# ml-unito/PartitionedLS.jl

Measured on NVIDIA B200. Metric: opt_fit_orthant_nnls_solves_per_sec, higher is better.
Workload: dtype f64

## Files before the change

partitionedls.jl_b200/csrc/nnls5.cu:

```cuda
#include "common.cuh"

namespace pls {
namespace {

constexpr int H5_BYTES_ = 192;
constexpr int SG_FREE5 = 2;
constexpr unsigned char ST_INO = 1;
constexpr unsigned char ST_PAS = 2;
constexpr unsigned char ST_BLK = 4;
constexpr unsigned char ST_FAST = 8;
#define SYNC5() __syncthreads()

__device__ __forceinline__ void dmma5(double &d0, double &d1, double a, double b) {
  asm("mma.sync.aligned.m8n8k4.row.col.f64.f64.f64.f64 {%0,%1}, {%2}, {%3}, {%0,%1};\n"
      : "+d"(d0), "+d"(d1) : "d"(a), "d"(b));
}
__device__ __forceinline__ double rcp5(double x) {
  double r;
  asm("rcp.approx.ftz.f64 %0, %1;" : "=d"(r) : "d"(x));
  double e = fma(-x, r, 1.0);
  r = fma(r, e, r);
  e = fma(-x, r, 1.0);
  return fma(r, e, r);
}
__device__ __forceinline__ double wsum5(double v) {
#pragma unroll
  for (int o = 16; o; o >>= 1) v += __shfl_xor_sync(0xffffffffu, v, o);
  return v;
}
__device__ __forceinline__ double wmax5(double v) {
#pragma unroll
  for (int o = 16; o; o >>= 1) v = fmax(v, __shfl_xor_sync(0xffffffffu, v, o));
  return v;
}
__host__ __device__ constexpr int t2_doubles(int nr) { return ((nr / 8) * (nr / 8 + 1) / 2) * 64; }
__device__ __forceinline__ int t2_idx(int i, int j) {
  const int ti = i >> 3, tj = j >> 3;
  return ((((ti * (ti + 1)) >> 1) + tj) << 6) + ((i & 7) << 3) + (j & 7);
}
__device__ __forceinline__ double t2_get(const double *T2, int i, int j) { return i >= j ? T2[t2_idx(i, j)] : T2[t2_idx(j, i)]; }
__device__ __forceinline__ void t2_set(double *T2, int i, int j, double v) {
  const int a = i > j ? i : j, b = i > j ? j : i;
  const int x = t2_idx(a, b);
  T2[x] = v;
  if ((a >> 3) == (b >> 3)) T2[x - ((a & 7) << 3) - (b & 7) + ((b & 7) << 3) + (a & 7)] = v;
}
__device__ __forceinline__ int pan5(int row, int col) { return (row << 3) + (col ^ ((row & 2) << 1)); }

struct Sh5 {
  double *T2;
  double *v;
  double *Pp, *Wp;
  double *yv;
  double *D;
  double *gd;
  double *red;
  int4 *binfo;
  int *ctl;
  short *slot;
  short *rvar;
  short *lst;
  short *lstE;
  short *lstB;
  unsigned short *tmap;
  signed char *sg;
  unsigned char *st;
  unsigned char *grp;
  unsigned char *mk;
};
enum { C_NS = 0, C_OK, C_CNT, C_N, C_NJ, C_NP, C_NLV, C_FLAG };

__host__ __device__ inline size_t sh5_bytes(int NR, int ld1) {
  const int ntl = (NR / 8) * (NR / 8 + 1) / 2;
  return H5_BYTES_ + sizeof(double) * ((size_t)t2_doubles(NR) + ld1 + 16 * (size_t)NR + NR + 64 + 8 + 32 + 16) + sizeof(int) * 16 +
         sizeof(short) * (2 * (size_t)ld1 + 2 * (size_t)NR + 8 + ((ntl + 3) & ~3)) + 3 * (size_t)ld1 + NR + 16 + 16;
}

__device__ __forceinline__ Sh5 make_sh5(int NR, int ld1) {
  extern __shared__ __align__(16) unsigned char smem_raw5[];
  const int ntl = (NR / 8) * (NR / 8 + 1) / 2;
  Sh5 s;
  double *dp = reinterpret_cast<double *>(smem_raw5 + H5_BYTES_);
  s.T2 = dp; dp += t2_doubles(NR);
  s.Pp = dp; dp += 8 * NR;
  s.Wp = dp; dp += 8 * NR;
  s.yv = dp; dp += NR;
  s.D = dp; dp += 64;
  s.gd = dp; dp += 8;
  s.red = dp; dp += 32;
  s.binfo = reinterpret_cast<int4 *>(dp); dp += 16;
  int *ip = reinterpret_cast<int *>(dp);
  s.ctl = ip; ip += 16;
  short *sp = reinterpret_cast<short *>(ip);
  s.rvar = sp; sp += NR;
  s.lstE = sp; sp += NR;
  s.lstB = sp; sp += 8;
  s.tmap = reinterpret_cast<unsigned short *>(sp); sp += (ntl + 3) & ~3;
  s.mk = reinterpret_cast<unsigned char *>(sp);
  dp = reinterpret_cast<double *>(smem_raw5 + ((static_cast<int>(s.mk - smem_raw5) + NR + 15) & ~15));
  s.v = dp; dp += ld1;
  sp = reinterpret_cast<short *>(dp);
  s.slot = sp; sp += ld1;
  s.lst = sp; sp += ld1;
  signed char *cp = reinterpret_cast<signed char *>(sp);
  s.sg = cp; cp += ld1;
  s.st = reinterpret_cast<unsigned char *>(cp); cp += ld1;
  s.grp = reinterpret_cast<unsigned char *>(cp);
  return s;
}

struct H5 {
  double *T1;
  const double *T1r;
  double *Pg;
  const double *G;
  const unsigned long long *gmask;
  int ld1, nr, Mp, ldg;
  int cold_fused;
  int gen;
  int pad0, pad1;
  unsigned long long cnt[10];
  double yy, cmax;
  double max_viol;
};
enum { H_SWEEP = 0, H_STREAM, H_SUMS, H_SUMP2, H_ITER, H_BLK, H_REBUILD, H_FOLD, H_DRIFT, H_NOCONV };
constexpr int H5_BYTES = H5_BYTES_;
static_assert(sizeof(H5) <= H5_BYTES, "header size");
__device__ __forceinline__ H5 &hdr5() {
  extern __shared__ __align__(16) unsigned char smem_raw5[];
  return *reinterpret_cast<H5 *>(smem_raw5);
}

template <int T>
__device__ __forceinline__ double bmax5(const Sh5 &s, double v) {
  constexpr int NW = T / 32;
  v = wmax5(v);
  if ((threadIdx.x & 31) == 0) s.red[threadIdx.x >> 5] = v;
  SYNC5();
  double r = s.red[0];
#pragma unroll
  for (int i = 1; i < NW; ++i) r = fmax(r, s.red[i]);
  SYNC5();
  return r;
}

template <int T>
__device__ __forceinline__ void set_block5(const Sh5 &s, int nb, int slot) {
  const int tid = threadIdx.x;
  const H5 &h = hdr5();
  const int g = h.gen;
  if (g == 1) {
    #pragma unroll 1
    for (int k = tid; k < h.nr; k += T) s.mk[k] = 0;
    SYNC5();
  }
  if (tid < nb) {
    const int tc = slot >> 3, c7 = slot & 7;
    s.lstB[tid] = (short)slot;
    s.binfo[tid] = make_int4(slot, (tc << 6) + c7, (((tc * (tc + 1)) >> 1) << 6) + (c7 << 3), 0);
    s.mk[slot] = (unsigned char)g;
  }
}

template <int T, int NR>
__device__ __noinline__ int t2_block(int n, int nb, int nlv, bool test, bool flip) {
  H5 &h = hdr5();
  const int gen = h.gen;
  const Sh5 s = make_sh5(NR, h.ld1);
  constexpr int NW = T / 32;
  const int tid = threadIdx.x, lane = tid & 31, wid = tid >> 5;
  const int fr = lane >> 2, fk = lane & 3;
  const int ntr = (n + 7) >> 3;
  const short *B = s.lstB;
  if (tid >= 32 || T == 32) {
    constexpr int TG = T == 32 ? 32 : T - 32;
#pragma unroll 1
    for (int row = T == 32 ? tid : tid - 32; row < ntr * 8; row += TG) {
      const int tr = row >> 3, r7 = row & 7;
      const int rbase = (((tr * (tr + 1)) >> 1) << 6) + (r7 << 3), rowt = (tr << 6) + r7;
      const int sw = (row & 2) << 1, pb = row << 3;
#pragma unroll 1
      for (int q = 0; q < 8; ++q) {
        double val = 0.0;
        if (row < n && q < nb) { const int4 bi = s.binfo[q]; val = s.T2[row >= bi.x ? rbase + bi.y : bi.z + rowt]; }
        s.Pp[pb + (q ^ sw)] = val;
      }
    }
  }
  if (tid < 32) {
    if (lane < 8) {
      s.gd[lane] = (test && lane >= nlv && lane < nb) ? 1e-13 * __ldg(h.G + (size_t)h.ldg * s.rvar[B[lane]] + s.rvar[B[lane]]) : 0.0;
    }
    const int i = lane >> 2, j0 = (lane & 3) << 1;
    double e0 = (i < nb && j0 < nb) ? t2_get(s.T2, B[i], B[j0]) : (i == j0 ? 1.0 : 0.0);
    double e1 = (i < nb && j0 + 1 < nb) ? t2_get(s.T2, B[i], B[j0 + 1]) : (i == j0 + 1 ? 1.0 : 0.0);
    int bad = nb;
#pragma unroll 1
    for (int k = 0; k < nb; ++k) {
      __syncwarp();
      s.D[i * 8 + j0] = e0; s.D[i * 8 + j0 + 1] = e1;
      __syncwarp();
      const double pk0 = s.D[k * 8 + j0], pk1 = s.D[k * 8 + j0 + 1], cik = s.D[i * 8 + k], pkk = s.D[k * 8 + k];
      const bool good = k < nlv ? pkk < 0.0 : (test ? pkk > s.gd[k] : pkk > 0.0);
      if (!good && bad == nb) bad = k;
      const double d = rcp5(pkk), fct = cik * d;
      const bool rowk = i == k;
      double n0 = rowk ? pk0 * d : fma(-fct, pk0, e0);
      double n1 = rowk ? pk1 * d : fma(-fct, pk1, e1);
      if (j0 == k) n0 = rowk ? d : -fct;
      if (j0 + 1 == k) n1 = rowk ? d : -fct;
      e0 = n0; e1 = n1;
    }
    __syncwarp();
    s.D[i * 8 + j0] = e0; s.D[i * 8 + j0 + 1] = e1;
    if (lane == 0) s.ctl[C_OK] = bad == nb ? nb : (bad < nlv ? -1 : bad);
  }
  SYNC5();
  const int res = s.ctl[C_OK];
  if (tid == 0) h.gen = gen == 255 ? 1 : gen + 1;
  if (res != nb) { SYNC5(); return res; }
  #pragma unroll 1
  for (int ti = wid; ti < ntr; ti += NW) {
    double c0 = 0.0, c1 = 0.0;
    dmma5(c0, c1, s.Pp[pan5(ti * 8 + fr, fk)], s.D[fk * 8 + fr]);
    dmma5(c0, c1, s.Pp[pan5(ti * 8 + fr, 4 + fk)], s.D[(4 + fk) * 8 + fr]);
    *reinterpret_cast<double2 *>(s.Wp + pan5(ti * 8 + fr, 2 * fk)) = make_double2(c0, c1);
  }
  SYNC5();
  {
    const int ntl = (ntr * (ntr + 1)) >> 1;
    int q = (ntl * wid) / NW;
    const int q1 = (ntl * (wid + 1)) / NW;
    const int t0 = s.tmap[q];
    int ti = t0 >> 8, tj = t0 & 255;
    const int la0 = pan5(fr, fk), la1 = pan5(fr, 4 + fk);
    double2 *cp = reinterpret_cast<double2 *>(s.T2 + (q << 6) + fr * 8 + 2 * fk);
    const double *pw = s.Wp + (ti << 6), *pp = s.Pp + (tj << 6);
    double a0 = -pw[la0], a1 = -pw[la1];
#pragma unroll 1
    for (; q < q1; ++q) {
      double2 c0 = *cp;
      dmma5(c0.x, c0.y, a0, pp[la0]);
      dmma5(c0.x, c0.y, a1, pp[la1]);
      *cp = c0;
      cp += 32; pp += 64;
      if (++tj > ti) { ++ti; tj = 0; pp = s.Pp; pw += 64; a0 = -pw[la0]; a1 = -pw[la1]; }
    }
  }
  SYNC5();
#pragma unroll 1
  for (int row = tid; row < n; row += T) {
    if (s.mk[row] == (unsigned char)gen) continue;
    const int tr = row >> 3, r7 = row & 7;
    const int rbase = (((tr * (tr + 1)) >> 1) << 6) + (r7 << 3), rowt = (tr << 6) + r7;
    const int sw = (row & 2) << 1, pb = row << 3;
#pragma unroll 1
    for (int q = 0; q < nb; ++q) {
      const int4 bi = s.binfo[q];
      const int tc = bi.x >> 3;
      const double w0 = s.Wp[pb + (q ^ sw)];
      const double val = q < nlv ? -w0 : w0;
      if (tr >= tc) s.T2[rbase + bi.y] = val;
      if (tr <= tc) s.T2[bi.z + rowt] = val;
    }
  }
#pragma unroll 1
  for (int e = tid; e < 64; e += T) {
    const int i = e >> 3, j = e & 7;
    if (i < nb && j <= i) { const double val = s.D[i * 8 + j]; t2_set(s.T2, B[i], B[j], ((i < nlv) == (j < nlv)) ? -val : val); }
  }
  if (flip && tid < nb) s.st[s.rvar[B[tid]]] ^= ST_PAS;
  SYNC5();
  if (tid == 0) { h.cnt[H_SWEEP] += nb; h.cnt[H_SUMP2] += ((unsigned long long)(n * n) * nb) >> 2; }
  return nb;
}

template <int T, int NR>
__device__ __noinline__ bool t2_rebuild(int n) {
  const H5 &h = hdr5();
  const Sh5 s = make_sh5(NR, h.ld1);
  constexpr int NW = T / 32;
  const int tid = threadIdx.x, lane = tid & 31, wid = tid >> 5;
  #pragma unroll 1
  for (int i = wid; i < n; i += NW) {
    const double *row = h.T1r + (size_t)h.ld1 * s.rvar[i];
    #pragma unroll 1
    for (int j = lane; j <= i; j += 32) t2_set(s.T2, i, j, __ldcg(row + s.rvar[j]));
  }
  if (tid < 32) {
    int cnt = 0, nlv = 0;
    #pragma unroll 1
    for (int pass = 0; pass < 2; ++pass) {
      #pragma unroll 1
      for (int k0 = 1; k0 < n; k0 += 32) {
        const int k = k0 + lane;
        bool take = false;
        if (k < n) { const unsigned char f = s.st[s.rvar[k]]; const bool pas = f & ST_PAS, ino = f & ST_INO; take = pas != ino && (pass == 0 ? !pas : pas); }
        const unsigned bal = __ballot_sync(0xffffffffu, take);
        if (take) s.lst[cnt + __popc(bal & ((1u << lane) - 1))] = (short)k;
        cnt += __popc(bal);
      }
      if (pass == 0) nlv = cnt;
    }
    if (lane == 0) { s.ctl[C_CNT] = cnt; s.ctl[C_NLV] = nlv; }
  }
  SYNC5();
  const int cnt = s.ctl[C_CNT], nlv = s.ctl[C_NLV];
  #pragma unroll 1
  for (int q0 = 0; q0 < cnt; q0 += 8) {
    const int nb = min(8, cnt - q0);
    set_block5<T>(s, nb, tid < nb ? s.lst[q0 + tid] : 0);
    SYNC5();
    if (t2_block<T, NR>(n, nb, max(0, min(nb, nlv - q0)), false, false) != nb) return false;
  }
  return true;
}

template <int NR>
__device__ __noinline__ int window_reset() {
  const H5 &h = hdr5();
  const Sh5 s = make_sh5(NR, h.ld1);
  const int tid = threadIdx.x;
  const int Mp = h.Mp;
  if (tid < 32) {
    const int lane = tid;
    if (lane == 0) s.rvar[0] = (short)Mp;
    int base = 1;
    #pragma unroll 1
    for (int m0 = 0; m0 < Mp; m0 += 32) {
      const int m = m0 + lane;
      bool keep = false;
      if (m < Mp) {
        const unsigned char f = s.st[m];
        keep = (f & ST_FAST) || (((f & ST_PAS) != 0) != ((f & ST_INO) != 0));
      }
      const unsigned bal = __ballot_sync(0xffffffffu, keep);
      if (m < Mp) {
        if (keep) { const int k = base + __popc(bal & ((1u << lane) - 1)); s.rvar[k] = (short)m; s.slot[m] = (short)k; }
        else s.slot[m] = -1;
      }
      base += __popc(bal);
    }
    if (lane == 0) s.ctl[C_N] = base;
  }
  SYNC5();
  return s.ctl[C_N];
}

template <int T, int NR>
__device__ __noinline__ int t2_compact(int n) {
  const H5 &h = hdr5();
  const Sh5 s = make_sh5(NR, h.ld1);
  const int tid = threadIdx.x;
  double *scr = h.Pg + 8 * (size_t)h.ld1;
  short *old = s.lst;
  if (tid < 32) {
    const int lane = tid;
    if (lane == 0) old[0] = 0;
    int base = 1;
    #pragma unroll 1
    for (int k0 = 1; k0 < n; k0 += 32) {
      const int k = k0 + lane;
      bool keep = false; int m = 0;
      if (k < n) {
        m = s.rvar[k];
        const unsigned char f = s.st[m];
        keep = (f & ST_FAST) || (((f & ST_PAS) != 0) != ((f & ST_INO) != 0));
      }
      const unsigned bal = __ballot_sync(0xffffffffu, keep);
      const int kn = base + __popc(bal & ((1u << lane) - 1));
      __syncwarp();
      if (k < n) {
        if (keep) { old[kn] = (short)k; s.rvar[kn] = (short)m; s.slot[m] = (short)kn; }
        else s.slot[m] = -1;
      }
      __syncwarp();
      base += __popc(bal);
    }
    if (lane == 0) s.ctl[C_N] = base;
  }
  SYNC5();
  const int nn = s.ctl[C_N];
  if (nn == n) return n;
  #pragma unroll 1
  for (int idx = tid; idx < nn * nn; idx += T) {
    const int a = idx / nn, b = idx - a * nn;
    if (b <= a) __stcg(scr + idx, t2_get(s.T2, old[a], old[b]));
  }
  __threadfence_block();
  SYNC5();
  #pragma unroll 1
  for (int idx = tid; idx < nn * nn; idx += T) {
    const int a = idx / nn, b = idx - a * nn;
    if (b <= a) t2_set(s.T2, a, b, __ldcg(scr + idx));
  }
  SYNC5();
// ... 212 lines not shown
          __stcg(reinterpret_cast<double2 *>(h.T1 + (size_t)(ri[u] * 8 + fr) * ld1 + rj[u] * 8 + 2 * fk), c[u]);
          if (ri[u] != rj[u]) {
            double *mp = h.T1 + (size_t)(rj[u] * 8 + 2 * fk) * ld1 + ri[u] * 8 + fr;
            __stcg(mp, c[u].x); __stcg(mp + ld1, c[u].y);
          }
        }
      }
    }
  }
  SYNC5();
  #pragma unroll 1
  for (int idx = tid; idx < ld1 * 8; idx += T) {
    const int i = idx >> 3, q = idx & 7;
    if (q < nb) {
      const double val = (s.st[B[q]] & ST_PAS) ? FW[pan5(i, q)] : -FW[pan5(i, q)];
      __stcg(h.T1 + (size_t)ld1 * B[q] + i, val);
      __stcg(h.T1 + (size_t)ld1 * i + B[q], val);
    }
  }
  SYNC5();
  #pragma unroll 1
  for (int e = tid; e < 64; e += T) {
    const int i = e >> 3, j = e & 7;
    if (i < nb && j < nb) {
      const double ei = (s.st[B[i]] & ST_PAS) ? 1.0 : -1.0, ej = (s.st[B[j]] & ST_PAS) ? 1.0 : -1.0;
      __stcg(h.T1 + (size_t)ld1 * B[i] + B[j], -ei * ej * s.D[i * 8 + j]);
    }
  }
  SYNC5();
  if (tid < nb) { const int m = B[tid]; const unsigned char f = s.st[m]; s.st[m] = (f & ST_PAS) ? (unsigned char)(f | ST_INO) : (unsigned char)(f & ~ST_INO); }
  if (tid == 0) { h.T1r = h.T1; h.cnt[H_SUMP2] += 2ull * ld1 * ld1; h.cnt[H_FOLD]++; }
  SYNC5();
  return true;
}

template <int T, int NR>
__device__ __noinline__ void fold_fused5(int n) {
  H5 &h = hdr5();
  const Sh5 s = make_sh5(NR, h.ld1);
  constexpr int NW = T / 32;
  const int tid = threadIdx.x, lane = tid & 31, wid = tid >> 5;
  const int fr = lane >> 2, fk = lane & 3;
  const int ld1 = h.ld1, nt = ld1 >> 3;
  const int ntr = (n + 7) >> 3, nk = ntr << 3;
  double *PR = h.Pg + 8 * (size_t)ld1, *ZT = PR + (size_t)ld1 * h.nr;
  int *roff = reinterpret_cast<int *>(s.Wp);
  const bool own = h.T1r == h.T1;
  const double *rows = own ? PR : h.T1r;
  #pragma unroll 1
  for (int k = tid; k < nk; k += T) {
    double e = 0.0;
    if (k >= 1 && k < n) { const unsigned char f = s.st[s.rvar[k]]; const bool pas = f & ST_PAS, ino = f & ST_INO; if (pas != ino) e = pas ? 1.0 : -1.0; }
    s.yv[k] = e;
    roff[k] = e != 0.0 ? (own ? k : (int)s.rvar[k]) * ld1 : 0;
  }
  SYNC5();
  if (own) {
    #pragma unroll 1
    for (int k = 0; k < n; ++k) {
      if (k > 0 && s.yv[k] == 0.0) continue;
      const double *src = h.T1 + (size_t)ld1 * (s.yv[k] != 0.0 ? s.rvar[k] : 0);
      #pragma unroll 1
      for (int j = tid; j < ld1; j += T) PR[(size_t)k * ld1 + j] = __ldcg(src + j);
    }
    __threadfence_block();
    SYNC5();
  }
  constexpr int NTQ = 12;
#pragma unroll 1
  for (int tj = wid; tj < nt; tj += NW) {
    const double *pa = rows + tj * 8 + fr;
    double2 acc[NTQ];
#pragma unroll
    for (int u = 0; u < NTQ; ++u) acc[u] = make_double2(0.0, 0.0);
    double a0 = s.yv[fk] * __ldcg(pa + roff[fk]), a1 = s.yv[4 + fk] * __ldcg(pa + roff[4 + fk]);
#pragma unroll 1
    for (int tk = 0; tk < ntr; ++tk) {
      double n0 = 0.0, n1 = 0.0;
      if (tk + 1 < ntr) { const int k = (tk + 1) * 8 + fk; n0 = s.yv[k] * __ldcg(pa + roff[k]); n1 = s.yv[k + 4] * __ldcg(pa + roff[k + 4]); }
#pragma unroll
      for (int tq = 0; tq < NTQ; ++tq) {
        if (tq < ntr) {
          double b0, b1;
          if (tk >= tq) { const double *tp = s.T2 + ((((tk * (tk + 1)) >> 1) + tq) << 6); b0 = tp[fk * 8 + fr]; b1 = tp[(4 + fk) * 8 + fr]; }
          else { const double *tp = s.T2 + ((((tq * (tq + 1)) >> 1) + tk) << 6); b0 = tp[fr * 8 + fk]; b1 = tp[fr * 8 + 4 + fk]; }
          dmma5(acc[tq].x, acc[tq].y, a0, b0); dmma5(acc[tq].x, acc[tq].y, a1, b1);
        }
      }
      a0 = n0; a1 = n1;
    }
#pragma unroll
    for (int tq = 0; tq < NTQ; ++tq)
      if (tq < ntr) {
        const int k = tq * 8 + 2 * fk;
        *reinterpret_cast<double2 *>(ZT + (size_t)(tj * 8 + fr) * nk + k) = make_double2(acc[tq].x * s.yv[k], acc[tq].y * s.yv[k + 1]);
      }
  }
  __threadfence_block();
  SYNC5();
  constexpr int CH = 5;
  {
    const int ntl = (nt * (nt + 1)) >> 1;
    int q = (ntl * wid) / NW;
    const int q1 = (ntl * (wid + 1)) / NW;
    int ti = 0;
    while (((ti + 1) * (ti + 2)) >> 1 <= q) ++ti;
    int tj = q - ((ti * (ti + 1)) >> 1);
    #pragma unroll 1
    for (; q < q1; ++q) {
      double2 c = __ldcg(reinterpret_cast<const double2 *>(h.T1r + (size_t)(ti * 8 + fr) * ld1 + tj * 8 + 2 * fk));
      const double *za = ZT + (size_t)(ti * 8 + fr) * nk + fk, *pb = rows + tj * 8 + fr;
#pragma unroll 1
      for (int t0 = 0; t0 < ntr; t0 += CH) {
        double z0[CH], z1[CH], p0[CH], p1[CH];
#pragma unroll
        for (int u = 0; u < CH; ++u) {
          const bool live = t0 + u < ntr;
          const int k = (t0 + u) * 8 + fk;
          z0[u] = live ? za[(t0 + u) * 8] : 0.0; z1[u] = live ? za[(t0 + u) * 8 + 4] : 0.0;
          p0[u] = live ? __ldcg(pb + roff[k]) : 0.0; p1[u] = live ? __ldcg(pb + roff[k + 4]) : 0.0;
        }
#pragma unroll
        for (int u = 0; u < CH; ++u) { dmma5(c.x, c.y, z0[u], p0[u]); dmma5(c.x, c.y, z1[u], p1[u]); }
      }
      __stcg(reinterpret_cast<double2 *>(h.T1 + (size_t)(ti * 8 + fr) * ld1 + tj * 8 + 2 * fk), c);
      if (ti != tj) {
        double *mp = h.T1 + (size_t)(tj * 8 + 2 * fk) * ld1 + ti * 8 + fr;
        __stcg(mp, c.x); __stcg(mp + ld1, c.y);
      }
      if (++tj > ti) { ++ti; tj = 0; }
    }
  }
  SYNC5();
  #pragma unroll 1
  for (int k = 1; k < n; ++k) {
    const double e = s.yv[k];
    if (e == 0.0) continue;
    const int var = s.rvar[k];
    #pragma unroll 1
    for (int j = tid; j < ld1; j += T) {
      const double val = -e * ZT[(size_t)j * nk + k];
      __stcg(h.T1 + (size_t)ld1 * var + j, val);
      __stcg(h.T1 + (size_t)ld1 * j + var, val);
    }
  }
  SYNC5();
  #pragma unroll 1
  for (int idx = tid; idx < n * n; idx += T) {
    const int a = idx / n, b = idx - a * n;
    __stcg(h.T1 + (size_t)ld1 * s.rvar[a] + s.rvar[b], t2_get(s.T2, a, b));
  }
  SYNC5();
  #pragma unroll 1
  for (int k = tid; k < n; k += T) {
    if (k >= 1 && s.yv[k] != 0.0) { const int m = s.rvar[k]; const unsigned char f = s.st[m]; s.st[m] = (f & ST_PAS) ? (unsigned char)(f | ST_INO) : (unsigned char)(f & ~ST_INO); }
  }
  if (tid == 0) { h.T1r = h.T1; h.cnt[H_SUMP2] += 2ull * ld1 * ld1 * (unsigned long long)ntr / 8 + (unsigned long long)ld1 * nk * nk / 2; h.cnt[H_FOLD]++; }
  SYNC5();
}

template <int T, int NR>
__device__ __noinline__ int fold5(int n, bool cold_mode) {
  const H5 &h = hdr5();
  const Sh5 s = make_sh5(NR, h.ld1);
  const int tid = threadIdx.x;
  if (cold_mode) n = t2_compact<T, NR>(n);
  short *B = s.lstE;
  if (tid < 32) {
// ... 64 lines not shown
      a0 = fma(-h.G[(size_t)h.ldg * s.lst[t] + m], wf[t], a0);
      a1 = fma(-h.G[(size_t)h.ldg * s.lst[t + 1] + m], wf[t + 1], a1);
    }
    if (t < np) a0 = fma(-h.G[(size_t)h.ldg * s.lst[t] + m], wf[t], a0);
    const double rv = a0 + a1;
    const int sg = s.sg[m];
    const unsigned char f = s.st[m];
    if (f & ST_PAS) mx = fmax(mx, fabs(rv));
    else if (sg == SG_FREE5) mx = fmax(mx, fabs(rv));
    else if (sg != 0 && !(f & ST_BLK)) mx = fmax(mx, (double)sg * rv);
  }
  return bmax5<T>(s, mx);
}

template <int T, int NR, int NQ>
__device__ __forceinline__ bool solve5(const Sh5 s, int &n_win, bool cold_mode, bool &t2_fresh) {
  const int tid = threadIdx.x;
  H5 &h = hdr5();
  const int Mp = h.Mp;
  const double cmax = h.cmax;
  const double told = 1e-12 * cmax;
  int t_best = Mp + 1, pbar = 3, iters = 0, rebuilt = 0;
  #pragma unroll 1
  for (;;) {
    #pragma unroll 1
    for (;;) {
      const int n = n_win;
      int nl = 0, ne = 0, mx = -1;
      {
        constexpr int NW = T / 32;
        const int lane = tid & 31, wid = tid >> 5;
        int4 *ri = reinterpret_cast<int4 *>(s.red);
        #pragma unroll 1
        for (int k0 = 1; k0 < n; k0 += T) {
          const int k = k0 + tid;
          int f = 0, m = -1;
          if (k < n) {
            m = s.rvar[k];
            const double val = s.T2[t2_idx(k, 0)];
            const int sg = s.sg[m];
            const unsigned char fl = s.st[m];
            if (fl & ST_PAS) { if (sg != SG_FREE5 && (sg == 0 || (double)sg * val < 0.0)) f = 1; }
            else if (!(fl & ST_BLK) && sg != 0 && (sg == SG_FREE5 ? fabs(val) > told : (double)sg * val > told)) f = 2;
          }
          const unsigned bl = __ballot_sync(0xffffffffu, f == 1), be = __ballot_sync(0xffffffffu, f == 2);
          const int mw = __reduce_max_sync(0xffffffffu, f ? m : -1);
          if (k0 > 1) SYNC5();
          if (lane == 0) ri[wid] = make_int4(__popc(bl), __popc(be), mw, 0);
          SYNC5();
          int ol = nl, oe = ne;
#pragma unroll
          for (int w2 = 0; w2 < NW; ++w2) {
            const int4 r = ri[w2];
            if (w2 < wid) { ol += r.x; oe += r.y; }
            nl += r.x; ne += r.y; mx = max(mx, r.z);
          }
          const unsigned below = (1u << lane) - 1;
          if (f == 1) s.lst[ol + __popc(bl & below)] = (short)k;
          if (f == 2) s.lstE[oe + __popc(be & below)] = (short)k;
        }
      }
      SYNC5();
      const int nv = nl + ne;
      if (nv == 0) break;
      if (tid == 0) h.cnt[H_ITER]++;
      if (++iters > 60 + 6 * Mp) return false;
      bool single = false;
      if (nv < t_best) { t_best = nv; pbar = 3; }
      else if (pbar >= 1) --pbar;
      else single = true;
      if (single) {
        const int k = s.slot[mx];
        const bool pas = s.st[mx] & ST_PAS;
        nl = pas ? 1 : 0; ne = pas ? 0 : 1;
        SYNC5();
        if (tid == 0) { if (pas) s.lst[0] = (short)k; else s.lstE[0] = (short)k; }
        SYNC5();
      }
      t2_fresh = false;
      int done = 0, tot = nl + ne;
      bool broken = false;
      while (done < tot) {
        const int nb = min(8, tot - done), nlv = max(0, min(nb, nl - done));
        set_block5<T>(s, nb, tid < nb ? (done + tid < nl ? s.lst[done + tid] : s.lstE[done + tid - nl]) : 0);
        SYNC5();
        const int r = t2_block<T, NR>(n, nb, nlv, true, true);
        if (r == nb) { done += nb; continue; }
        if (r < 0) { broken = true; break; }
        const int pos = done + r - nl;
        if (tid == 0) {
          s.st[s.rvar[s.lstE[pos]]] |= ST_BLK;
          #pragma unroll 1
          for (int q = pos; q + 1 < ne; ++q) s.lstE[q] = s.lstE[q + 1];
        }
        --ne; --tot; if (tid == 0) h.cnt[H_BLK]++;
        SYNC5();
      }
      if (broken) {
        if (++rebuilt > 3 || !t2_rebuild<T, NR>(n)) return false;
        t2_fresh = true; if (tid == 0) h.cnt[H_REBUILD]++;
      }
    }
    stream5<T, NQ, NR>(n_win);
    {
      const int ns = s.ctl[C_NS];
      int code = 0;
#pragma unroll 1
      for (int p = tid; p < ns; p += T) if (!(fabs(s.v[s.lst[p]]) <= 1e-12 * cmax)) code |= 2;
#pragma unroll 1
      for (int m = tid; m < Mp; m += T) {
        if (s.slot[m] < 0) {
          const int sg = s.sg[m];
          const unsigned char fl = s.st[m];
          const double val = s.v[m];
          bool f;
          if (fl & ST_INO) f = sg != SG_FREE5 && (sg == 0 ? val != 0.0 : (double)sg * val < 0.0);
          else f = !(fl & ST_BLK) && sg != 0 && (sg == SG_FREE5 ? fabs(val) > told : (double)sg * val > told);
          if (f) code |= 1;
        }
      }
      if (code) atomicOr(&s.ctl[C_FLAG], code);
      SYNC5();
      const int flags = s.ctl[C_FLAG];
      if (flags & 2) {
        double res = 0.0;
#pragma unroll 1
        for (int p = tid; p < ns; p += T) { const double r = fabs(s.v[s.lst[p]]); res = r == r ? fmax(res, r) : r; }
        res = bmax5<T>(s, res);
        if (res != res || (t2_fresh && res > 1e-9 * cmax) || ++rebuilt > 3) return false;
        if (!t2_rebuild<T, NR>(n_win)) return false;
        t2_fresh = true;
        if (tid == 0) h.cnt[H_REBUILD]++;
        continue;
      }
      if (!(flags & 1)) return true;
    }
    if (tid < 32) {
      const int lane = tid;
      int nj = 0;
#pragma unroll 1
      for (int m0 = 0; m0 < Mp; m0 += 32) {
        const int m = m0 + lane;
        bool f = false;
        if (m < Mp && s.slot[m] < 0) {
          const int sg = s.sg[m];
          const unsigned char fl = s.st[m];
          const double val = s.v[m];
          if (fl & ST_INO) f = sg != SG_FREE5 && (sg == 0 ? val != 0.0 : (double)sg * val < 0.0);
          else f = !(fl & ST_BLK) && sg != 0 && (sg == SG_FREE5 ? fabs(val) > told : (double)sg * val > told);
        }
        const unsigned bal = __ballot_sync(0xffffffffu, f);
        if (f) s.lst[nj + __popc(bal & ((1u << lane) - 1))] = (short)m;
        nj += __popc(bal);
      }
      if (lane == 0) s.ctl[C_NJ] = nj;
    }
    SYNC5();
    const int nj = s.ctl[C_NJ];
    if (nj == 0) return true;
    if (++iters > 60 + 6 * Mp) return false;
    if (NR - n_win < nj) {
      short *park = reinterpret_cast<short *>(s.v);
      #pragma unroll 1
      for (int p = tid; p < nj; p += T) park[p] = s.lst[p];
      SYNC5();
      if (cold_mode) n_win = t2_compact<T, NR>(n_win);
      if (NR - n_win < (nj < 8 ? nj : 8)) {
        const int nf = fold5<T, NR>(n_win, cold_mode);
        if (nf < 0) return false;
        n_win = nf;
        t2_fresh = true;
      }
      int room = NR - n_win;
      if (room > nj) room = nj;
      if (room <= 0) return false;
      #pragma unroll 1
      for (int p = 0; p < room; ++p) { const int m = park[p]; if (s.slot[m] < 0) { join5<T, NR>(n_win, m); ++n_win; } }
    } else {
      #pragma unroll 1
      for (int p = 0; p < nj; ++p) { join5<T, NR>(n_win, s.lst[p]); ++n_win; }
    }
    t_best = Mp + 1; pbar = 3;
  }
}

template <int T, int NR>
__device__ __noinline__ void cold_init5(const double *T0) {
  H5 &h = hdr5();
  const Sh5 s = make_sh5(NR, h.ld1);
  const int tid = threadIdx.x, ld1 = h.ld1;
  if (tid == 0) h.T1r = T0;
  #pragma unroll 1
  for (int m = tid; m < ld1; m += T) { s.st[m] = 0; s.slot[m] = -1; s.sg[m] = 0; }
  SYNC5();
}

__global__ void __launch_bounds__(128) k2v5_build_t0(const double *G, int ldg, const double *c, const double *scal, int Mp, int ld1, double *T0) {
  const int row = blockIdx.x;
  for (int col = threadIdx.x; col < ld1; col += blockDim.x) {
    double val = 0.0;
    if (row < Mp) val = col < Mp ? G[(size_t)ldg * row + col] : (col == Mp ? c[row] : 0.0);
    else if (row == Mp) val = col < Mp ? c[col] : (col == Mp ? scal[0] : 0.0);
    T0[(size_t)ld1 * row + col] = val;
  }
}

template <int T>
__device__ __forceinline__ void set_lowmask5(const Sh5 &s, unsigned long long mask) {
  const H5 &h = hdr5();
  #pragma unroll 1
  for (int m = threadIdx.x; m < h.Mp; m += T) {
    const unsigned char f = s.st[m];
    s.st[m] = (h.gmask[m] & mask) ? (unsigned char)(f | ST_FAST) : (unsigned char)(f & ~ST_FAST);
  }
  SYNC5();
}

template <int T>
__device__ __forceinline__ void set_signs5(const Sh5 &s, long long b, int free_top, int Kp, int fb) {
  const H5 &h = hdr5();
  #pragma unroll 1
  for (int m = threadIdx.x; m < h.Mp; m += T) {
    const int g = s.grp[m];
    if (fb >= 0 && g != 255) {
      if (g == fb) s.sg[m] = (signed char)-s.sg[m];
    } else if (fb < 0 || ((h.gmask[m] >> fb) & 1ull)) {
      const unsigned long long gm = h.gmask[m];
      const int d = 2 * __popcll(gm & (unsigned long long)b) - __popcll(gm);
      const bool fr = free_top && ((gm >> (Kp - 1)) & 1ull);
      s.sg[m] = (signed char)(fr ? SG_FREE5 : (d > 0) - (d < 0));
    }
    s.st[m] &= (unsigned char)~ST_BLK;
  }
  SYNC5();
}

template <int T, int NR, int NQ, int MINB>
__global__ void __launch_bounds__(T, MINB) k2v5_orthant_walks(const K2Args A) {
  const int tid = threadIdx.x;
  const int Mp = A.Mp, ld1 = A.cap;
  const Sh5 s = make_sh5(NR, ld1);
  H5 &h = hdr5();
  if (tid == 0) {
    h.T1 = A.tab + (size_t)blockIdx.x * A.tabstride; h.ld1 = ld1; h.T1r = A.hglob;
    h.Pg = h.T1 + (size_t)ld1 * ld1;
    h.Mp = Mp; h.nr = NR; h.cold_fused = A.chain_log2; h.gen = 1;
    h.gmask = reinterpret_cast<const unsigned long long *>(A.gmask);
    h.G = A.G; h.ldg = A.ldg;
    #pragma unroll 1
    for (int q = 0; q < 10; ++q) h.cnt[q] = 0;
    h.yy = A.scal[0]; h.cmax = A.scal[1]; h.max_viol = 0.0;
  }
  int n_win = 1;
  bool cold_mode = true;
  #pragma unroll 1
  for (int ti = tid; ti < NR / 8; ti += T)
    #pragma unroll 1
    for (int tj = 0; tj <= ti; ++tj) s.tmap[((ti * (ti + 1)) >> 1) + tj] = (unsigned short)((ti << 8) | tj);
  #pragma unroll 1
  for (int k = tid; k < NR; k += T) s.mk[k] = 0;
  #pragma unroll 1
  for (int m = tid; m < Mp; m += T) { const unsigned long long gm = reinterpret_cast<const unsigned long long *>(A.gmask)[m]; s.grp[m] = (unsigned char)(__popcll(gm) == 1 ? __ffsll((long long)gm) - 1 : 255); }
  #pragma unroll 1
  for (int e = tid; e < t2_doubles(NR); e += T) s.T2[e] = 0.0;
  double best_obj = 0.0; long long best_b = -1;
  int low_bits = 0;
  while ((A.lowmask >> low_bits) & 1ull) ++low_bits;
  const long long cnt = A.n_chains;
  const long long i0 = cnt * (long long)blockIdx.x / (long long)gridDim.x;
  const long long i1 = cnt * ((long long)blockIdx.x + 1) / (long long)gridDim.x;
  bool cold = true, just_cold = false, t2_fresh = true;
  int since_check = 0, check_every = A.verify_every;
  SYNC5();

  #pragma unroll 1
  for (long long i = i0; i < i1; ++i) {
    if (cold) {
      cold_init5<T, NR>(A.hglob);
      cold_mode = true;
      n_win = window_reset<NR>();
      t2_rebuild<T, NR>(n_win);
      cold = false; just_cold = true; since_check = 0; t2_fresh = true;
    }
    const long long b = A.b_begin + (i ^ (i >> 1));
    const int fb = i > 0 ? __ffsll(i) - 1 : 63;
    set_signs5<T>(s, b, A.free_top, A.Kp, (just_cold || i == i0) ? -1 : fb);

    const bool ok = solve5<T, NR, NQ>(s, n_win, cold_mode, t2_fresh);
    if (!ok) { cold = true; if (tid == 0) h.cnt[H_NOCONV]++; }

    ++since_check;
    if (ok && (since_check >= check_every || i + 1 == i1)) {
      since_check = 0;
      const double viol = verify5<T, NR>(A.c);
      const double cmax = h.cmax;
      if (!just_cold && tid == 0) h.max_viol = fmax(h.max_viol, viol);
      if (viol > 1e-13 * cmax && check_every > 8) check_every = 8;
      if (viol > 1e-12 * cmax && !just_cold) { if (tid == 0) h.cnt[H_DRIFT]++; cold = true; --i; continue; }
    }
    just_cold = false;

    const double obj = ok ? sqrt(fmax(s.v[Mp], 0.0)) : __longlong_as_double(0x7ff8000000000000ll);
    const long long rel = b - A.b_begin;
    double w_top = 0.0;
    if (A.free_top && (s.st[Mp - 1] & ST_PAS)) w_top = s.slot[Mp - 1] >= 0 ? s.T2[t2_idx(s.slot[Mp - 1], 0)] : s.v[Mp - 1];
    const long long b_full = A.free_top ? (b | ((w_top > 0.0 ? 1ll : 0ll) << (A.Kp - 1))) : b;
    if (A.all_obj && tid == 0) A.all_obj[rel] = obj;
    const bool better = opt_better(obj, b_full, best_obj, best_b, PLS_TIE_REL * h.yy);
    if (better) { best_obj = obj; best_b = b_full; }
    if (A.all_alpha || better) {
      #pragma unroll 1
      for (int m = tid; m < Mp; m += T) {
        const unsigned long long gm = h.gmask[m];
        const int d = 2 * __popcll(gm & (unsigned long long)b) - __popcll(gm);
        double wv = 0.0;
        if (ok && (s.st[m] & ST_PAS)) wv = s.slot[m] >= 0 ? s.T2[t2_idx(s.slot[m], 0)] : s.v[m];
        const double al = s.sg[m] == SG_FREE5 ? fabs(wv) : (d != 0 ? fmax(wv / (double)d, 0.0) : 0.0);
        if (A.all_alpha) A.all_alpha[(size_t)rel * Mp + m] = al;
        if (better) A.cta_w[(size_t)blockIdx.x * Mp + m] = al;
      }
    }
    if (ok) {
      bool tslow = false;
#pragma unroll 1
      for (int k = tid + 1; k < n_win; k += T) {
        const int m = s.rvar[k]; const unsigned char f = s.st[m];
        tslow = tslow || ((((f & ST_PAS) != 0) != ((f & ST_INO) != 0)) && !(f & ST_FAST));
      }
      const int nslow = __syncthreads_count(tslow);
      const bool was_cold = cold_mode;
      if (fb >= low_bits || nslow >= 8 || n_win > NR - 8 || was_cold) {
        const int nf = fold5<T, NR>(n_win, cold_mode);
        if (nf < 0) cold = true;
        else n_win = nf;
        t2_fresh = true;
        if (was_cold && !cold) {
          set_lowmask5<T>(s, A.lowmask);
          cold_mode = false;
          n_win = window_reset<NR>();
          if (!t2_rebuild<T, NR>(n_win)) cold = true;
        }
      }
    }
// ... 90 lines not shown
```

Measured before the change: 35.40 million.

## Pack pivot block slots into registers and fuse W panel into rank update

Drops the shared-memory block info, block list and generation marker arrays. Each thread now packs the up-to-8 block slot indices into two 32-bit registers and uses byte-compare intrinsics for membership tests, which removes the set_block pass and a block-wide barrier per pivot block. The separate W = P·D tensor-core pass and its barrier are folded into the triangular rank-update loop, so each warp computes a W tile lazily when it reaches a new row and syncs only within the warp. The trade-off is that W tiles may be recomputed by several warps and slot lookups now take extra integer arithmetic. Slot indices are also assumed to fit in a byte.

```diff
diff --git a/partitionedls.jl_b200/csrc/nnls5.cu b/partitionedls.jl_b200/csrc/nnls5.cu
--- a/partitionedls.jl_b200/csrc/nnls5.cu
+++ b/partitionedls.jl_b200/csrc/nnls5.cu
@@ -34,16 +34,17 @@
   return v;
 }
 __host__ __device__ constexpr int t2_doubles(int nr) { return ((nr / 8) * (nr / 8 + 1) / 2) * 64; }
+__device__ __forceinline__ int t2_off(int r7, int c7) { return (r7 << 3) + c7; }
 __device__ __forceinline__ int t2_idx(int i, int j) {
   const int ti = i >> 3, tj = j >> 3;
-  return ((((ti * (ti + 1)) >> 1) + tj) << 6) + ((i & 7) << 3) + (j & 7);
+  return ((((ti * (ti + 1)) >> 1) + tj) << 6) + t2_off(i & 7, j & 7);
 }
 __device__ __forceinline__ double t2_get(const double *T2, int i, int j) { return i >= j ? T2[t2_idx(i, j)] : T2[t2_idx(j, i)]; }
 __device__ __forceinline__ void t2_set(double *T2, int i, int j, double v) {
   const int a = i > j ? i : j, b = i > j ? j : i;
   const int x = t2_idx(a, b);
   T2[x] = v;
-  if ((a >> 3) == (b >> 3)) T2[x - ((a & 7) << 3) - (b & 7) + ((b & 7) << 3) + (a & 7)] = v;
+  if ((a >> 3) == (b >> 3)) T2[x - t2_off(a & 7, b & 7) + t2_off(b & 7, a & 7)] = v;
 }
 __device__ __forceinline__ int pan5(int row, int col) { return (row << 3) + (col ^ ((row & 2) << 1)); }
 
@@ -55,25 +56,22 @@
   double *D;
   double *gd;
   double *red;
-  int4 *binfo;
   int *ctl;
   short *slot;
   short *rvar;
   short *lst;
   short *lstE;
-  short *lstB;
   unsigned short *tmap;
   signed char *sg;
   unsigned char *st;
   unsigned char *grp;
-  unsigned char *mk;
 };
 enum { C_NS = 0, C_OK, C_CNT, C_N, C_NJ, C_NP, C_NLV, C_FLAG };
 
 __host__ __device__ inline size_t sh5_bytes(int NR, int ld1) {
   const int ntl = (NR / 8) * (NR / 8 + 1) / 2;
-  return H5_BYTES_ + sizeof(double) * ((size_t)t2_doubles(NR) + ld1 + 16 * (size_t)NR + NR + 64 + 8 + 32 + 16) + sizeof(int) * 16 +
-         sizeof(short) * (2 * (size_t)ld1 + 2 * (size_t)NR + 8 + ((ntl + 3) & ~3)) + 3 * (size_t)ld1 + NR + 16 + 16;
+  return H5_BYTES_ + sizeof(double) * ((size_t)t2_doubles(NR) + ld1 + 16 * (size_t)NR + NR + 64 + 8 + 32) + sizeof(int) * 16 +
+         sizeof(short) * (2 * (size_t)ld1 + 2 * (size_t)NR + ((ntl + 3) & ~3)) + 3 * (size_t)ld1 + 16 + 16 + (144 + NR);
 }
 
 __device__ __forceinline__ Sh5 make_sh5(int NR, int ld1) {
@@ -88,16 +86,13 @@
   s.D = dp; dp += 64;
   s.gd = dp; dp += 8;
   s.red = dp; dp += 32;
-  s.binfo = reinterpret_cast<int4 *>(dp); dp += 16;
   int *ip = reinterpret_cast<int *>(dp);
   s.ctl = ip; ip += 16;
   short *sp = reinterpret_cast<short *>(ip);
   s.rvar = sp; sp += NR;
   s.lstE = sp; sp += NR;
-  s.lstB = sp; sp += 8;
   s.tmap = reinterpret_cast<unsigned short *>(sp); sp += (ntl + 3) & ~3;
-  s.mk = reinterpret_cast<unsigned char *>(sp);
-  dp = reinterpret_cast<double *>(smem_raw5 + ((static_cast<int>(s.mk - smem_raw5) + NR + 15) & ~15));
+  dp = reinterpret_cast<double *>(smem_raw5 + ((static_cast<int>(reinterpret_cast<unsigned char *>(sp) - smem_raw5) + 15) & ~15));
   s.v = dp; dp += ld1;
   sp = reinterpret_cast<short *>(dp);
   s.slot = sp; sp += ld1;
@@ -117,8 +112,7 @@
   const unsigned long long *gmask;
   int ld1, nr, Mp, ldg;
   int cold_fused;
-  int gen;
-  int pad0, pad1;
+  int pad0, pad1, pad2;
   unsigned long long cnt[10];
   double yy, cmax;
   double max_viol;
@@ -144,56 +138,53 @@
   return r;
 }
 
-template <int T>
-__device__ __forceinline__ void set_block5(const Sh5 &s, int nb, int slot) {
-  const int tid = threadIdx.x;
-  const H5 &h = hdr5();
-  const int g = h.gen;
-  if (g == 1) {
-    #pragma unroll 1
-    for (int k = tid; k < h.nr; k += T) s.mk[k] = 0;
-    SYNC5();
-  }
-  if (tid < nb) {
-    const int tc = slot >> 3, c7 = slot & 7;
-    s.lstB[tid] = (short)slot;
-    s.binfo[tid] = make_int4(slot, (tc << 6) + c7, (((tc * (tc + 1)) >> 1) << 6) + (c7 << 3), 0);
-    s.mk[slot] = (unsigned char)g;
-  }
-}
-
+__device__ __forceinline__ int bslot5(unsigned blo, unsigned bhi, int q) { return ((q < 4 ? blo : bhi) >> ((q & 3) << 3)) & 255; }
+__device__ __forceinline__ int bpos5(unsigned blo, unsigned bhi, int x) {
+  const unsigned xx = (unsigned)x * 0x01010101u;
+  const unsigned long long m = ((unsigned long long)__vcmpeq4(bhi, xx) << 32) | __vcmpeq4(blo, xx);
+  return m ? (__ffsll((long long)m) - 1) >> 3 : -1;
+}
 template <int T, int NR>
-__device__ __noinline__ int t2_block(int n, int nb, int nlv, bool test, bool flip) {
+__device__ __noinline__ int t2_block(int n, int nb, int nlv, int done, int nl, bool test, bool flip) {
   H5 &h = hdr5();
-  const int gen = h.gen;
   const Sh5 s = make_sh5(NR, h.ld1);
   constexpr int NW = T / 32;
   const int tid = threadIdx.x, lane = tid & 31, wid = tid >> 5;
   const int fr = lane >> 2, fk = lane & 3;
   const int ntr = (n + 7) >> 3;
-  const short *B = s.lstB;
+  unsigned blo = 0xffffffffu, bhi = 0xffffffffu;
+#pragma unroll 1
+  for (int q = 0; q < nb; ++q) {
+    const int p = done + q;
+    const unsigned k = (unsigned)(p < nl ? s.lst[p] : s.lstE[p - nl]);
+    if (q < 4) blo ^= (k ^ 255u) << (q << 3); else bhi ^= (k ^ 255u) << ((q - 4) << 3);
+  }
   if (tid >= 32 || T == 32) {
     constexpr int TG = T == 32 ? 32 : T - 32;
 #pragma unroll 1
     for (int row = T == 32 ? tid : tid - 32; row < ntr * 8; row += TG) {
       const int tr = row >> 3, r7 = row & 7;
-      const int rbase = (((tr * (tr + 1)) >> 1) << 6) + (r7 << 3), rowt = (tr << 6) + r7;
+      const int rbase = ((tr * (tr + 1)) >> 1) << 6, rowt = tr << 6;
       const int sw = (row & 2) << 1, pb = row << 3;
 #pragma unroll 1
       for (int q = 0; q < 8; ++q) {
         double val = 0.0;
-        if (row < n && q < nb) { const int4 bi = s.binfo[q]; val = s.T2[row >= bi.x ? rbase + bi.y : bi.z + rowt]; }
+        if (row < n && q < nb) {
+          const int c = bslot5(blo, bhi, q), tc = c >> 3, c7 = c & 7;
+          val = s.T2[row >= c ? rbase + (tc << 6) + t2_off(r7, c7) : (((tc * (tc + 1)) >> 1) << 6) + rowt + t2_off(c7, r7)];
+        }
         s.Pp[pb + (q ^ sw)] = val;
       }
     }
   }
   if (tid < 32) {
     if (lane < 8) {
-      s.gd[lane] = (test && lane >= nlv && lane < nb) ? 1e-13 * __ldg(h.G + (size_t)h.ldg * s.rvar[B[lane]] + s.rvar[B[lane]]) : 0.0;
+      s.gd[lane] = (test && lane >= nlv && lane < nb) ? 1e-13 * __ldg(h.G + (size_t)h.ldg * s.rvar[bslot5(blo, bhi, lane)] + s.rvar[bslot5(blo, bhi, lane)]) : 0.0;
     }
     const int i = lane >> 2, j0 = (lane & 3) << 1;
-    double e0 = (i < nb && j0 < nb) ? t2_get(s.T2, B[i], B[j0]) : (i == j0 ? 1.0 : 0.0);
-    double e1 = (i < nb && j0 + 1 < nb) ? t2_get(s.T2, B[i], B[j0 + 1]) : (i == j0 + 1 ? 1.0 : 0.0);
+    const int bi = bslot5(blo, bhi, i);
+    double e0 = (i < nb && j0 < nb) ? t2_get(s.T2, bi, bslot5(blo, bhi, j0)) : (i == j0 ? 1.0 : 0.0);
+    double e1 = (i < nb && j0 + 1 < nb) ? t2_get(s.T2, bi, bslot5(blo, bhi, j0 + 1)) : (i == j0 + 1 ? 1.0 : 0.0);
     int bad = nb;
 #pragma unroll 1
     for (int k = 0; k < nb; ++k) {
@@ -217,59 +208,62 @@
   }
   SYNC5();
   const int res = s.ctl[C_OK];
-  if (tid == 0) h.gen = gen == 255 ? 1 : gen + 1;
   if (res != nb) { SYNC5(); return res; }
-  #pragma unroll 1
-  for (int ti = wid; ti < ntr; ti += NW) {
-    double c0 = 0.0, c1 = 0.0;
-    dmma5(c0, c1, s.Pp[pan5(ti * 8 + fr, fk)], s.D[fk * 8 + fr]);
-    dmma5(c0, c1, s.Pp[pan5(ti * 8 + fr, 4 + fk)], s.D[(4 + fk) * 8 + fr]);
-    *reinterpret_cast<double2 *>(s.Wp + pan5(ti * 8 + fr, 2 * fk)) = make_double2(c0, c1);
-  }
-  SYNC5();
   {
     const int ntl = (ntr * (ntr + 1)) >> 1;
     int q = (ntl * wid) / NW;
     const int q1 = (ntl * (wid + 1)) / NW;
-    const int t0 = s.tmap[q];
-    int ti = t0 >> 8, tj = t0 & 255;
-    const int la0 = pan5(fr, fk), la1 = pan5(fr, 4 + fk);
-    double2 *cp = reinterpret_cast<double2 *>(s.T2 + (q << 6) + fr * 8 + 2 * fk);
-    const double *pw = s.Wp + (ti << 6), *pp = s.Pp + (tj << 6);
-    double a0 = -pw[la0], a1 = -pw[la1];
-#pragma unroll 1
-    for (; q < q1; ++q) {
-      double2 c0 = *cp;
-      dmma5(c0.x, c0.y, a0, pp[la0]);
-      dmma5(c0.x, c0.y, a1, pp[la1]);
-      *cp = c0;
-      cp += 32; pp += 64;
-      if (++tj > ti) { ++ti; tj = 0; pp = s.Pp; pw += 64; a0 = -pw[la0]; a1 = -pw[la1]; }
+    if (q < q1) {
+      const int t0 = s.tmap[q];
+      int ti = t0 >> 8, tj = t0 & 255;
+      const int la0 = pan5(fr, fk), la1 = pan5(fr, 4 + fk);
+      const double d0 = s.D[fk * 8 + fr], d1 = s.D[(4 + fk) * 8 + fr];
+      double2 *cp = reinterpret_cast<double2 *>(s.T2 + (q << 6) + t2_off(fr, 2 * fk));
+      const double *pp = s.Pp + (tj << 6);
+      double a0, a1;
+#pragma unroll 1
+      for (bool newrow = true; q < q1; ++q) {
+        if (newrow) {
+          double w0 = 0.0, w1 = 0.0;
+          dmma5(w0, w1, s.Pp[pan5(ti * 8 + fr, fk)], d0);
+          dmma5(w0, w1, s.Pp[pan5(ti * 8 + fr, 4 + fk)], d1);
+          double *pw = s.Wp + (ti << 6);
+          *reinterpret_cast<double2 *>(pw + pan5(fr, 2 * fk)) = make_double2(w0, w1);
+          __syncwarp();
+          a0 = -pw[la0]; a1 = -pw[la1];
+          newrow = false;
+        }
+        double2 c0 = *cp;
+        dmma5(c0.x, c0.y, a0, pp[la0]);
+        dmma5(c0.x, c0.y, a1, pp[la1]);
+        *cp = c0;
+        cp += 32; pp += 64;
+        if (++tj > ti) { ++ti; tj = 0; pp = s.Pp; newrow = true; }
+      }
     }
   }
   SYNC5();
 #pragma unroll 1
   for (int row = tid; row < n; row += T) {
-    if (s.mk[row] == (unsigned char)gen) continue;
+    if (bpos5(blo, bhi, row) >= 0) continue;
     const int tr = row >> 3, r7 = row & 7;
-    const int rbase = (((tr * (tr + 1)) >> 1) << 6) + (r7 << 3), rowt = (tr << 6) + r7;
+    const int rbase = ((tr * (tr + 1)) >> 1) << 6, rowt = tr << 6;
     const int sw = (row & 2) << 1, pb = row << 3;
 #pragma unroll 1
     for (int q = 0; q < nb; ++q) {
-      const int4 bi = s.binfo[q];
-      const int tc = bi.x >> 3;
+      const int c = bslot5(blo, bhi, q), tc = c >> 3, c7 = c & 7;
       const double w0 = s.Wp[pb + (q ^ sw)];
       const double val = q < nlv ? -w0 : w0;
-      if (tr >= tc) s.T2[rbase + bi.y] = val;
-      if (tr <= tc) s.T2[bi.z + rowt] = val;
+      if (tr >= tc) s.T2[rbase + (tc << 6) + t2_off(r7, c7)] = val;
+      if (tr <= tc) s.T2[(((tc * (tc + 1)) >> 1) << 6) + rowt + t2_off(c7, r7)] = val;
     }
   }
 #pragma unroll 1
   for (int e = tid; e < 64; e += T) {
     const int i = e >> 3, j = e & 7;
-    if (i < nb && j <= i) { const double val = s.D[i * 8 + j]; t2_set(s.T2, B[i], B[j], ((i < nlv) == (j < nlv)) ? -val : val); }
-  }
-  if (flip && tid < nb) s.st[s.rvar[B[tid]]] ^= ST_PAS;
+    if (i < nb && j <= i) { const double val = s.D[i * 8 + j]; t2_set(s.T2, bslot5(blo, bhi, i), bslot5(blo, bhi, j), ((i < nlv) == (j < nlv)) ? -val : val); }
+  }
+  if (flip && tid < nb) s.st[s.rvar[bslot5(blo, bhi, tid)]] ^= ST_PAS;
   SYNC5();
   if (tid == 0) { h.cnt[H_SWEEP] += nb; h.cnt[H_SUMP2] += ((unsigned long long)(n * n) * nb) >> 2; }
   return nb;
@@ -309,9 +303,7 @@
   #pragma unroll 1
   for (int q0 = 0; q0 < cnt; q0 += 8) {
     const int nb = min(8, cnt - q0);
-    set_block5<T>(s, nb, tid < nb ? s.lst[q0 + tid] : 0);
-    SYNC5();
-    if (t2_block<T, NR>(n, nb, max(0, min(nb, nlv - q0)), false, false) != nb) return false;
+    if (t2_block<T, NR>(n, nb, max(0, min(nb, nlv - q0)), q0, cnt, false, false) != nb) return false;
   }
   return true;
 }
@@ -690,8 +682,8 @@
       for (int tq = 0; tq < NTQ; ++tq) {
         if (tq < ntr) {
           double b0, b1;
-          if (tk >= tq) { const double *tp = s.T2 + ((((tk * (tk + 1)) >> 1) + tq) << 6); b0 = tp[fk * 8 + fr]; b1 = tp[(4 + fk) * 8 + fr]; }
-          else { const double *tp = s.T2 + ((((tq * (tq + 1)) >> 1) + tk) << 6); b0 = tp[fr * 8 + fk]; b1 = tp[fr * 8 + 4 + fk]; }
+          if (tk >= tq) { const double *tp = s.T2 + ((((tk * (tk + 1)) >> 1) + tq) << 6); b0 = tp[t2_off(fk, fr)]; b1 = tp[t2_off(4 + fk, fr)]; }
+          else { const double *tp = s.T2 + ((((tq * (tq + 1)) >> 1) + tk) << 6); b0 = tp[t2_off(fr, fk)]; b1 = tp[t2_off(fr, 4 + fk)]; }
           dmma5(acc[tq].x, acc[tq].y, a0, b0); dmma5(acc[tq].x, acc[tq].y, a1, b1);
         }
       }
@@ -922,9 +914,7 @@
       bool broken = false;
       while (done < tot) {
         const int nb = min(8, tot - done), nlv = max(0, min(nb, nl - done));
-        set_block5<T>(s, nb, tid < nb ? (done + tid < nl ? s.lst[done + tid] : s.lstE[done + tid - nl]) : 0);
-        SYNC5();
-        const int r = t2_block<T, NR>(n, nb, nlv, true, true);
+        const int r = t2_block<T, NR>(n, nb, nlv, done, nl, true, true);
         if (r == nb) { done += nb; continue; }
         if (r < 0) { broken = true; break; }
         const int pos = done + r - nl;
@@ -1084,7 +1074,7 @@
   if (tid == 0) {
     h.T1 = A.tab + (size_t)blockIdx.x * A.tabstride; h.ld1 = ld1; h.T1r = A.hglob;
     h.Pg = h.T1 + (size_t)ld1 * ld1;
-    h.Mp = Mp; h.nr = NR; h.cold_fused = A.chain_log2; h.gen = 1;
+    h.Mp = Mp; h.nr = NR; h.cold_fused = A.chain_log2;
     h.gmask = reinterpret_cast<const unsigned long long *>(A.gmask);
     h.G = A.G; h.ldg = A.ldg;
     #pragma unroll 1
@@ -1097,8 +1087,6 @@
   for (int ti = tid; ti < NR / 8; ti += T)
     #pragma unroll 1
     for (int tj = 0; tj <= ti; ++tj) s.tmap[((ti * (ti + 1)) >> 1) + tj] = (unsigned short)((ti << 8) | tj);
-  #pragma unroll 1
-  for (int k = tid; k < NR; k += T) s.mk[k] = 0;
   #pragma unroll 1
   for (int m = tid; m < Mp; m += T) { const unsigned long long gm = reinterpret_cast<const unsigned long long *>(A.gmask)[m]; s.grp[m] = (unsigned char)(__popcll(gm) == 1 ? __ffsll((long long)gm) - 1 : 255); }
   #pragma unroll 1
```

Measured after the change: 34.22 million (median of 6 runs). 0.967x the previous value.
